# CaptainEven/DenseBox

Measured on AMD Instinct MI355X. Metric: training patches/sec (240x240), higher is better.
Workload: dtype f16; 1 GPU; full training step (fwd + fused dense loss w/ hard-negative mining + bwd + grad all-reduce + SGD) of DenseBoxLMLOC on 240x240 patches; net=DenseBoxLMLOC, batch_per_gpu=64, global_batch=64, patch=240x240, parallelism=dp1, half_neg=11, grad_finite=True

## Files before the change

densebox_amd/_lib.py:

```python
import ctypes as C
import os

_HERE = os.path.dirname(os.path.abspath(__file__))
LIB_PATH = os.environ.get('DBX_LIB') or os.path.join(_HERE, 'csrc', 'libdensebox_hip.so')

F16, BF16, F32 = 0, 1, 2
DTYPE_ID = {'f16': F16, 'bf16': BF16, 'f32': F32}
ESIZE = {F16: 2, BF16: 2, F32: 4}

EPI_BIAS, EPI_RELU, EPI_GATE, EPI_DROPMASK, EPI_ACCUM, EPI_F32_NCHW, EPI_DROPHASH = 1, 2, 4, 8, 16, 32, 64
CONV_WFRAG = 128
K_IGEMM, K_DMA, K_BAND, K_C64, K_C8, K_WS, K_P8 = 1, 2, 3, 4, 5, 6, 7


class View(C.Structure):
    _fields_ = [('ptr', C.c_void_p), ('n', C.c_int32), ('h', C.c_int32), ('w', C.c_int32),
                ('pad', C.c_int32), ('ld', C.c_int32), ('c_off', C.c_int32), ('c', C.c_int32)]


class ConvDesc(C.Structure):
    _fields_ = [('dtype', C.c_int32), ('kh', C.c_int32), ('kw', C.c_int32), ('cpad', C.c_int32),
                ('cin_pad', C.c_int32), ('cout_pad', C.c_int32), ('epilogue', C.c_int32), ('drop_seed', C.c_uint32)]


# ... 88 lines not shown
    'dbx_dp_destroy': (C.c_int, [_VP]),
    'dbx_conv_dgrad_wgrad1_scratch_bytes': (_I64, []),
    'dbx_conv_dgrad_wgrad1_fusable': (C.c_int, [_PC, _PV, _PV, _PV]),
    'dbx_conv_dgrad_wgrad1': (C.c_int, [_PC, _PV, _VP, _PV, _PV, _I32, _VP, _VP, _VP, _I32, _VP]),
    'dbx_conv_pool_fusable': (C.c_int, [_PC, _PV, _PV]),
    'dbx_conv_forward_pool': (C.c_int, [_PC, _PV, _VP, _VP, _PV, _PV, _I32, _VP]),
    'dbx_conv_forward_pool_idx': (C.c_int, [_PC, _PV, _VP, _VP, _PV, _PV, _I32, _VP, _VP]),
    'dbx_pack_weight': (C.c_int, [_I32, _I32, _VP, _I32, _I32, _I32, _I32, _VP, _I32, _I32, _I32, _I32, _VP]),
    'dbx_fold_heads': (C.c_int, [_VP, _VP, _VP, _VP, _I32, _VP, _VP, _VP]),
    'dbx_fold_refine': (C.c_int, [_VP, _VP, _VP, _VP, _VP, _VP, _I32, _I32, _VP, _VP, _VP, _VP]),
    'dbx_refine_eval': (C.c_int, [_VP, _VP, _I32, _I32, _I32, _VP, _VP, _VP, _VP]),
    'dbx_refine_backward_scratch_bytes': (C.c_int64, [_I32, _I32, _I32]),
    'dbx_refine_backward': (C.c_int, [_VP, _VP, _VP, _I32, _I32, _I32, _VP, _VP, _VP, _VP, _VP, _VP, _I32, _VP, _VP, _VP, _VP, _VP, _VP, _VP, _VP, _VP, _VP, _VP, _VP, _VP, _VP]),
    'dbx_upsample_bilinear_nchw_f32': (C.c_int, [_VP, _I32, _I32, _I32, _VP, _I32, _I32, _VP]),
    'dbx_pack_multi': (C.c_int, [_I32, _VP, _I32, _I64, _VP]),
    'dbx_sgd_pack_step': (C.c_int, [_I32, _VP, _I32, _I64, _VP, _F, _F, _F, _I32, _VP]),
    'dbx_head2_dgrad': (C.c_int, [_I32, _PV, C.POINTER(C.c_void_p), C.POINTER(C.c_int32), _I32, _PV, _VP, _I32, _I32, C.c_uint32, _VP]),
    'dbx_head2_wgrad_scratch_bytes': (_I64, [_I32, _I32]),
    'dbx_head2_wgrad': (C.c_int, [_I32, _PV, _PV, C.POINTER(C.c_int32), _I32, C.POINTER(C.c_void_p), C.POINTER(C.c_void_p), _VP, _VP]),
    'dbx_head2_backward': (C.c_int, [_I32, _PV, _PV, C.POINTER(C.c_void_p), C.POINTER(C.c_int32), _I32, _PV, _VP, _I32, _I32, C.c_uint32,
                                     C.POINTER(C.c_void_p), C.POINTER(C.c_void_p), _VP, _VP]),
    'dbx_head2_backward_up': (C.c_int, [_I32, _PV, _PV, C.POINTER(C.c_void_p), C.POINTER(C.c_int32), _I32, _PV, _VP, _I32, _I32, C.c_uint32,
                                        C.POINTER(C.c_void_p), C.POINTER(C.c_void_p), _VP, _PV, _VP]),
    'dbx_perspective_matrix': (C.c_int, [_VP, _VP, _VP]),
    'dbx_warp_perspective_u8': (C.c_int, [_VP, _I32, _I32, _I32, _VP, _VP, _I32, _I32, _VP]),
    'dbx_warp_batch_workspace_bytes': (_I64, [_I32]),
    'dbx_warp_perspective_batch_u8': (C.c_int, [C.POINTER(WarpJob), _I32, _I32, _VP, _VP, _VP]),
    'dbx_plate_crops_batch': (C.c_int, [_VP, _I32, _I32, _VP, _I64, _I64, _VP, _I32, _I32, _I32, _VP, _VP, _VP, _VP]),
    'dbx_match_gt_batch': (C.c_int, [_VP, _I32, _I64, _VP, _VP, _I32, _I32, _VP, _I32, _VP, _VP, _I32, _D, _VP, _VP, _VP, _VP, _VP, _VP]),
    'dbx_eval_append': (C.c_int, [_VP, _I32, _I64, _VP, _VP, _I32, _I32, _VP, _VP, _VP, _VP, _I64, _VP, _VP]),
    'dbx_track_update_batch': (C.c_int, [_VP, _I32, _I64, _VP, _VP, _I32, _I32, _VP, _VP, _I32, _I32, _I32, _D, _I32, _D, _D, _D, _VP, _VP, _VP,
                                         _VP, _VP, _VP]),
    'dbx_track_append': (C.c_int, [_VP, _VP, _I32, _I32, _I32, _VP, _I64, _VP, _VP]),
    'dbx_crop_sharpness': (C.c_int, [_VP, _I64, _I32, _I32, _I32, _VP, _VP]),
    'dbx_track_gallery_update': (C.c_int, [_VP, _VP, _VP, _VP, _VP, _VP, _VP, _VP, _VP, _VP, _VP, _VP, _VP, _I32, _I32, _I32, _I32, _I32, _I32,
                                           _I32, _I32, _I64, _I32, _D, _I32, _VP]),
    'dbx_draw_overlay_batch': (C.c_int, [_VP, _I32, _I32, _I32, _I32, _VP, _I32, _I64, _VP, _VP, _I32, _VP, _VP, _VP, _I32, _I32,
                                         C.POINTER(OverlayStyle), _VP]),
    'dbx_overlay_font': (C.c_int, [_VP]),
    'dbx_overlay_label': (C.c_int, [_D, _I32, C.c_char_p, _I32]),
    'dbx_resize_batch_workspace_bytes': (_I64, [_I32]),
    'dbx_resize_cubic_batch_u8': (C.c_int, [C.POINTER(ResizeJob), _I32, _I32, _VP, _VP, _VP]),
    'dbx_conv_wgrad_scratch_bytes': (_I64, [_I32, _PV, _PV, _I32, _I32]),
    'dbx_conv_wgrad': (C.c_int, [_I32, _PV, _PV, _I32, _I32, _I32, _I32, _I32, _VP, _VP, _VP, _I32, _VP]),
    'dbx_conv_wgrad_slice': (C.c_int, [_I32, _PV, _PV, _I32, _I32, _I32, _I32, _I32, _VP, _I32, _I32, _VP, _VP, _I32, _VP]),
    'dbx_conv_wgrad_pool_dz_ok': (C.c_int, [_I32, _PV, _PV, _I32, _I32]),
# ... 91 lines not shown
```

densebox_amd/csrc/aux_ops.hip:

```cpp
#include "common.hpp"
#include <mutex>

static thread_local char g_err[512] = "";
void dbx_set_error(const char* fmt, ...) {
    va_list ap;
    va_start(ap, fmt);
    vsnprintf(g_err, sizeof(g_err), fmt, ap);
    va_end(ap);
}
extern "C" const char* dbx_last_error(void) { return g_err; }
extern "C" int dbx_version(void) { return DBX_ABI_VERSION; }
extern "C" int dbx_device_arch(int device) {
    hipDeviceProp_t p;
    if (hipGetDeviceProperties(&p, device) != hipSuccess) { dbx_set_error("hipGetDeviceProperties failed"); return DBX_ERR_HIP; }
    int arch = 0;
    const char* s = p.gcnArchName;
    if (s[0] == 'g' && s[1] == 'f' && s[2] == 'x') arch = (int)strtol(s + 3, nullptr, 16) == 0x950 ? 950 : (int)strtol(s + 3, nullptr, 10);
    return arch;
}

template <typename T> struct Vec { static constexpr int N = 16 / sizeof(T); };

template <typename T> __device__ __forceinline__ void load_vec(const T* p, float (&v)[16 / sizeof(T)]) {
    const u32x4 raw = *(const u32x4*)p;
// ... 1036 lines not shown
extern "C" int dbx_head2_backward(int32_t dtype, const dbx_view* d_out, const dbx_view* hid, const float* const* w2, const int32_t* k,
                                  int32_t nh, const dbx_view* d_hid, const uint8_t* dropmask, int32_t dropmask_ld, int32_t use_hash,
                                  uint32_t drop_seed, float* const* dw, float* const* db, void* scratch, void* stream) {
    if (!d_out || !hid || !w2 || !k || !d_hid || !dw || !scratch) { dbx_set_error("head2_backward: null argument"); return DBX_ERR_ARG; }
    DBX_DISPATCH_DTYPE(dtype, head2_wgrad_t, d_out, hid, k, nh, dw, db, scratch, (hipStream_t)stream, w2, d_hid, dropmask, dropmask_ld,
                       use_hash, (unsigned)drop_seed);
}

#ifndef H2U_D
#define H2U_D 2
#endif
#ifndef H2U_NB
#define H2U_NB 4
#endif
#ifndef H2U_WGS
#define H2U_WGS 512
#endif
struct H2UHalf { int px_lo, px_n, own_lo, own_hi, ix_lo, ix_n; };
struct H2UPlan { int halves; H2UHalf h[2]; };
template <typename T, int KJ>
__global__ __launch_bounds__(256, 2) void head2_backward_up_kernel(FrameGeo dout, FrameGeo hid, FrameGeo dhid, FrameGeo dg, int hd0, int nhl, int slot,
                                                                   Head2Args ha, float* __restrict__ partial, float* __restrict__ bpartial,
                                                                   const unsigned char* __restrict__ mask, int mask_ld, int use_hash,
                                                                   unsigned drop_seed, float sy, float sx, H2UPlan plan, int nostore) {
    constexpr int V = 8, CS = 64, LPP = CS / V, D = H2U_D, PW = 32, NB = H2U_NB, NT = 6;
    static_assert(sizeof(T) == 2, "16-bit element types");
    __shared__ int s_x0[64], s_lo[32], s_hi[32];
    __shared__ float s_l0[64], s_l1[64];
    extern __shared__ __attribute__((aligned(16))) char h2u_smem[];
    float* const s_v = (float*)h2u_smem;
    const int nsl = nhl * (512 / CS), H = hid.h, W = hid.w;
    int b = blockIdx.x;
    const int sl = b % nsl; b /= nsl;
    const int half = b % plan.halves, grp = b / plan.halves, G = gridDim.x / (nsl * plan.halves);
    const H2UHalf hf = half ? plan.h[1] : plan.h[0];
    const int hd = hd0 + sl / (512 / CS), cbase = (sl % (512 / CS)) * CS;
    const int pl = threadIdx.x / LPP, ch = threadIdx.x % LPP, c0 = cbase + ch * V;
    const int px = hf.px_lo + pl;
    const bool active = pl < hf.px_n, owner = active && px >= hf.own_lo && px < hf.own_hi;
    if (threadIdx.x < W) {
        int x0, x1; float lx0, lx1;
        bilin_coef((int)threadIdx.x, sx, dg.w, x0, x1, lx0, lx1);
        s_x0[threadIdx.x] = x0; s_l0[threadIdx.x] = x1 == x0 ? lx0 + lx1 : lx0; s_l1[threadIdx.x] = x1 == x0 ? 0.f : lx1;
    }
    __syncthreads();
    if (threadIdx.x < hf.ix_n) {
        const int ix = hf.ix_lo + threadIdx.x;
// ... 206 lines not shown
            for (int j = 0; j < 8; ++j) red[4 * 8 * CS + wv * 8 + j] = j < KJ ? bs[j < KJ ? j : 0] : 0.f;
        }
    }
    __syncthreads();
    {
        const size_t blk = (size_t)grp * plan.halves + half;
        const int c = threadIdx.x % CS;
#pragma unroll
        for (int jj = 0; jj < 2; ++jj) {
            const int j = threadIdx.x / CS + 4 * jj;
            float o = 0.f;
#pragma unroll
            for (int q = 0; q < 4; ++q) o += red[(q * 8 + j) * CS + c];
            partial[(blk * nhl * 8 + (hd - hd0) * 8 + j) * 512 + cbase + c] = o;
        }
        if (cbase == 0 && threadIdx.x < 8) {
            float bsum = 0.f;
#pragma unroll
            for (int q = 0; q < 4; ++q) bsum += red[4 * 8 * CS + q * 8 + threadIdx.x];
            bpartial[blk * 32 + (hd - hd0) * 8 + threadIdx.x] = bsum;
        }
    }
}
static bool h2u_plan(int W, int ws, float sx, H2UPlan& p) {
    if (W > 64 || ws > 32 || W < 1 || ws < 1) return false;
    int x0[64];
    for (int ox = 0; ox < W; ++ox) { int v = (int)(sx * (float)ox); x0[ox] = v > ws - 1 ? ws - 1 : v; }
    if (W <= 32 && ws <= 16) { p.halves = 1; p.h[0] = p.h[1] = H2UHalf{0, W, 0, W, 0, ws}; return true; }
    const int S = ws / 2;
    if (S < 1 || S > 16 || ws - S > 16) return false;
    int hiL = -1, loR = W;
    for (int ox = 0; ox < W; ++ox) { if (x0[ox] <= S - 1) hiL = ox; if (x0[ox] >= S - 1 && ox < loR) loR = ox; }
    if (hiL + 1 > 32 || W - loR > 32 || loR > hiL + 1) return false;
    const int P = (loR + hiL + 1) / 2;
    p.halves = 2;
    p.h[0] = H2UHalf{0, hiL + 1, 0, P, 0, S};
    p.h[1] = H2UHalf{loR, W - loR, P, W, S, ws - S};
    return true;
}
template <typename T>
static int head2_backward_up_t(const dbx_view* dout, const dbx_view* hid, const float* const* w2, const int32_t* k, int nh, const dbx_view* dhid,
                               const uint8_t* mask, int mask_ld, int use_hash, unsigned drop_seed, float* const* dw, float* const* db,
                               void* scratch, const dbx_view* dg, hipStream_t s) {
    VIEW_VEC_CHECK(T, dg, "head2_backward_up d_g44");
    DBX_REQUIRE(dg->n == hid->n && dg->c == hid->c, "head2_backward_up: d_g44 has the hidden map's batch and channels");
    const float sy = ac_scale(dg->h, hid->h), sx = ac_scale(dg->w, hid->w);
    H2UPlan plan;
    bool fused = sizeof(T) == 2 && sy > 0.f && sy < 1.f && sx > 0.45f && sx < 1.f && hid->c % 64 == 0 && hid->h >= 2 && h2u_plan(hid->w, dg->w, sx, plan);
    if (const char* e = getenv("DBX_HEAD2_UP")) fused = fused && atoi(e) != 0;
    const bool nostore = dhid->ptr == nullptr;
    DBX_REQUIRE(!nostore || (fused && !mask), "head2_backward_up without d_hid: needs the one-pass kernel (dbx_head2_backward_up_fused) and hash / no dropout");
    if (!fused) {
        const int rc = head2_wgrad_t<T>(dout, hid, k, nh, dw, db, scratch, s, w2, dhid, mask, mask_ld, use_hash, drop_seed);
        return rc != DBX_OK ? rc : upsample_bwd_t<T>(dhid, dg, nullptr, s);
    }
    if constexpr (sizeof(T) == 2) {
        VIEW_VEC_CHECK(T, hid, "head2_backward_up hid");
        if (!nostore) VIEW_VEC_CHECK(T, dhid, "head2_backward_up d_hid");
        DBX_REQUIRE(nh >= 1 && nh <= 4 && hid->c == 512 * nh && dout->c % nh == 0 && dout->c / nh >= 8, "head2_backward_up: nh in 1..4, hid of 512*nh channels, d_out of nh slots >= 8 channels");
        DBX_REQUIRE(dout->n == hid->n && dout->h == hid->h && dout->w == hid->w && dhid->n == hid->n && dhid->h == hid->h && dhid->w == hid->w && dhid->c == hid->c,
                    "head2_backward_up: shape mismatch");
        DBX_REQUIRE(((size_t)dout->ptr % 16) == 0 && (dout->ld * sizeof(T)) % 16 == 0 && (dout->c_off * sizeof(T)) % 16 == 0 &&
                        ((dout->c / nh) * sizeof(T)) % 16 == 0, "head2_backward_up: d_out alignment");
        Head2Out o;
        Head2Args ha;
        ha.nh = nh; ha.slot = dout->c / nh;
        for (int i = 0; i < 4; ++i) {
            o.dw[i] = i < nh ? dw[i] : nullptr; o.db[i] = (i < nh && db) ? db[i] : nullptr; o.k[i] = i < nh ? k[i] : 0;
            ha.w2[i] = i < nh ? w2[i] : nullptr; ha.k[i] = i < nh ? k[i] : 0;
            if (i < nh) DBX_REQUIRE(k[i] >= 1 && k[i] <= 8 && dw[i] && w2[i] && ((size_t)w2[i] % 16) == 0, "head2_backward_up: k in 1..8, 16-byte aligned weights");
        }
        constexpr size_t smem = (size_t)2 * H2U_NB * 32 * 64 * 4;
        static_assert(smem >= (4 * 8 * 64 + 32) * 4 && 2 * smem + 4096 <= 160 * 1024, "LDS budget of two workgroups per CU");
        static DbxDevOnce attr_once; int attr_dev = 0;
        if (attr_once.pending(&attr_dev)) {
            DBX_HIP(hipFuncSetAttribute((const void*)head2_backward_up_kernel<T, 1>, hipFuncAttributeMaxDynamicSharedMemorySize, (int)smem));
            DBX_HIP(hipFuncSetAttribute((const void*)head2_backward_up_kernel<T, 2>, hipFuncAttributeMaxDynamicSharedMemorySize, (int)smem));
            DBX_HIP(hipFuncSetAttribute((const void*)head2_backward_up_kernel<T, 4>, hipFuncAttributeMaxDynamicSharedMemorySize, (int)smem));
            DBX_HIP(hipFuncSetAttribute((const void*)head2_backward_up_kernel<T, 8>, hipFuncAttributeMaxDynamicSharedMemorySize, (int)smem));
            attr_once.mark(attr_dev);
        }
        static int split = -1;
        if (split < 0) { const char* e = getenv("DBX_HEAD2_UP_SPLIT"); split = e ? atoi(e) : 1; }
        auto kup = [&](int kk) { return !split ? 8 : kk <= 1 ? 1 : kk <= 2 ? 2 : kk <= 4 ? 4 : 8; };
        float* const pbase = (float*)scratch;
        long long pused = 0;
        int blocks_max = 0;
        for (int h0 = 0; h0 < nh;) {
            int h1 = h0 + 1;
            while (h1 < nh && kup(k[h1]) == kup(k[h0])) ++h1;
            const int nhl = h1 - h0, nsl = nhl * 8, kj = kup(k[h0]);
            int groups = H2U_WGS / (nsl * plan.halves);
            groups = groups < 1 ? 1 : groups > hid->n ? hid->n : groups;
            const int blocks = groups * plan.halves;
            float* partial = pbase + pused;
            float* bpartial = partial + (size_t)blocks * nhl * 8 * 512;
            for (int i = h0; i < h1; ++i) { o.poff[i] = pused; o.boff[i] = pused + (long long)blocks * nhl * 8 * 512; o.nblk[i] = blocks; o.nhl[i] = nhl; o.hl[i] = i - h0; }
            pused += (long long)blocks * (nhl * 8 * 512 + 32);
            blocks_max = blocks > blocks_max ? blocks : blocks_max;
#define H2U_LAUNCH(KJ)                                                                                                              \
            hipLaunchKernelGGL((head2_backward_up_kernel<T, KJ>), dim3(blocks * nsl), dim3(256), smem, s, make_geo<T>(dout), make_geo<T>(hid),    \
                               make_geo<T>(nostore ? hid : dhid), make_geo<T>(dg), h0, nhl, dout->c / nh, ha, partial, bpartial, mask, mask_ld,    \
                               use_hash, drop_seed, sy, sx, plan, nostore ? 1 : 0)
            if (kj == 1) H2U_LAUNCH(1); else if (kj == 2) H2U_LAUNCH(2); else if (kj == 4) H2U_LAUNCH(4); else H2U_LAUNCH(8);
#undef H2U_LAUNCH
            DBX_LAUNCH_CHECK();
            h0 = h1;
        }
        for (int i = nh; i < 4; ++i) { o.poff[i] = 0; o.boff[i] = 0; o.nblk[i] = 0; o.nhl[i] = 1; o.hl[i] = 0; }
        float* partial = pbase; float* bpartial = pbase;
        const int blocks = blocks_max;
        const int total = nh * 8 * 512 + nh * 8;
        hipLaunchKernelGGL(head2_wgrad_reduce_kernel, dim3((total + 63) / 64), dim3(1024), 0, s, partial, bpartial, blocks, nh, o);
        DBX_LAUNCH_CHECK();
    }
    return DBX_OK;
}
template <typename T> static int head2_up_fused_t(const dbx_view* hid, const dbx_view* dg) {
    const float sy = ac_scale(dg->h, hid->h), sx = ac_scale(dg->w, hid->w);
    H2UPlan plan;
    bool fused = sizeof(T) == 2 && sy > 0.f && sy < 1.f && sx > 0.45f && sx < 1.f && hid->c % 64 == 0 && hid->h >= 2 && h2u_plan(hid->w, dg->w, sx, plan);
    if (const char* e = getenv("DBX_HEAD2_UP")) fused = fused && atoi(e) != 0;
    return fused ? 1 : 0;
}
extern "C" int dbx_head2_backward_up_fused(int32_t dtype, const dbx_view* hid, const dbx_view* d_g44) {
    if (!hid || !d_g44) return 0;
    switch (dtype) { case DBX_F16: return head2_up_fused_t<_Float16>(hid, d_g44); case DBX_BF16: return head2_up_fused_t<__bf16>(hid, d_g44); default: return 0; }
}
extern "C" int dbx_head2_backward_up(int32_t dtype, const dbx_view* d_out, const dbx_view* hid, const float* const* w2, const int32_t* k,
                                     int32_t nh, const dbx_view* d_hid, const uint8_t* dropmask, int32_t dropmask_ld, int32_t use_hash,
                                     uint32_t drop_seed, float* const* dw, float* const* db, void* scratch, const dbx_view* d_g44, void* stream) {
    if (!d_out || !hid || !w2 || !k || !d_hid || !dw || !scratch || !d_g44) { dbx_set_error("head2_backward_up: null argument"); return DBX_ERR_ARG; }
    DBX_DISPATCH_DTYPE(dtype, head2_backward_up_t, d_out, hid, w2, k, nh, d_hid, dropmask, dropmask_ld, use_hash, (unsigned)drop_seed, dw, db,
                       scratch, d_g44, (hipStream_t)stream);
}

struct PackJob { const float* src; void* dst; int co, ci, taps, mode; long long ktot; int cin_pad, row_off, k_off, rows_lim; };
template <typename T>
__global__ void pack_multi_kernel(const PackJob* __restrict__ jobs) {
    const PackJob j = jobs[blockIdx.y];
    const int total = j.co * j.ci * j.taps, taps = j.taps, ci = j.ci;
    T* wp = (T*)j.dst;
    const bool fwd = j.mode == 0 || j.mode == 4;
    const int rl = j.mode >= 4 ? (int)j.ktot : j.rows_lim;
    if (sizeof(T) == 2 && j.mode != 2 && (fwd ? ci : j.co) % 8 == 0 && (j.k_off & 7) == 0 && (j.cin_pad & 7) == 0 && taps <= 25) {
        __shared__ float tile[8][32 * 25];
        const int ot = (j.co + 7) / 8, ctn = (ci + 31) / 32, ntiles = ot * ctn, row_f = 32 * taps;
        for (int tl = blockIdx.x; tl < ntiles; tl += gridDim.x) {
            const int o0 = (tl / ctn) * 8, c0 = (tl % ctn) * 32;
            const int cw = min(32, ci - c0), ow = min(8, j.co - o0);
            __syncthreads();
            for (int e = threadIdx.x; e < 8 * row_f; e += blockDim.x) {
                const int r = e / row_f, f = e - r * row_f;
                tile[r][f] = (r < ow && f < cw * taps) ? j.src[((o0 + r) * ci + c0) * taps + f] : 0.f;
            }
            __syncthreads();
            const int nch = fwd ? 8 * taps * 4 : 32 * taps;
// ... 370 lines not shown
```

densebox_amd/engine.py:

```python
import ctypes as C
import os
import weakref

import torch

from . import _lib
from ._lib import View, ConvDesc, check, ptr, stream_ptr

_BACKBONE = [('conv1_1_1', 3, 64), ('conv1_2_1', 64, 64), ('conv2_1_1', 64, 128), ('conv2_2_1', 128, 128),
             ('conv3_1_1', 128, 256), ('conv3_2_1', 256, 256), ('conv3_4_1', 256, 256),
             ('conv4_1_1', 256, 512), ('conv4_2_1', 512, 512), ('conv4_3_1', 512, 512), ('conv4_4_1', 512, 512)]

_HEADS = {
    'DenseBox': [('det', 1), ('loc', 4)],
    'DenseBoxLM': [('det', 1), ('loc', 4), ('landmark', 4)],
    'DenseBoxLMLOC': [('det', 1), ('loc', 4), ('landmark', 4), ('lmloc', 8)],
}


_FWD_IO = {'conv1_1_1': ('x0', 'a11'), 'conv1_2_1': ('a11', 'a12'), 'conv2_1_1': ('p1', 'a21'), 'conv2_2_1': ('a21', 'a22'),
           'conv3_1_1': ('p2', 'a31'), 'conv3_2_1': ('a31', 'a32'), 'conv3_4_1': ('a32', 'c34'), 'conv4_1_1': ('p3', 'a41'),
           'conv4_2_1': ('a41', 'a42'), 'conv4_3_1': ('a42', 'a43'), 'conv4_4_1': ('a43', 'a44')}
_BWD_IO = {'conv4_4_1': ('d_a44', 'd_a43'), 'conv4_3_1': ('d_a43', 'd_a42'), 'conv4_2_1': ('d_a42', 'd_a41'),
           'conv4_1_1': ('d_a41', 'd_p3'), 'conv3_4_1': ('d_c34', 'd_a32'), 'conv3_2_1': ('d_a32', 'd_a31'),
# ... 1004 lines not shown
            dgrad('conv6_2_det', B['d_rf_2'].view(), B['d_rf_1'].view(), 5, 5, 4, 64, 64)
            conv_bwd('conv6_1_det', B['d_rf_1'].view(), B['rf_p'].view(), 3, 3, 0, 64, 5)
            dgrad('conv6_1_det', B['d_rf_1'].view(), B['d_rf_p'].view(), 3, 3, 2, 64, 64)
            check(L.dbx_maxpool2x2_bwd(dt, C.byref(B['rf_in'].view()), C.byref(B['d_rf_p'].view()),
                                       C.byref(B['d_rf_in'].view()), 0, 0, s))

        slot = {}
        srcs = []
        for i, (stem, k) in enumerate(heads):
            slot[stem] = B['d_out'].view(P.crf * i, P.crf)
            src = override.get(stem)
            srcs.append(src if src is not None else gout(stem, k))
        if override or kind == 'DenseBox':
            check(L.dbx_nchw_to_framed_slots(dt, (C.c_void_p * nh)(*[t.data_ptr() for t in srcs]), (C.c_int32 * nh)(*[k for _, k in heads]), nh, P.crf,
                                             C.byref(B['d_out'].view()), s))
        else:
            for (stem, k), t in zip(heads, srcs):
                check(L.dbx_nchw_to_framed(dt, ptr(t), k, C.byref(slot[stem]), s))
        if kind != 'DenseBox' and not override:
            check(L.dbx_framed_add_ch(dt, C.byref(B['d_rf_in'].view()), 0, 4, C.byref(slot['landmark']), 0, s))
            check(L.dbx_framed_add_ch(dt, C.byref(B['d_rf_in'].view()), 4, 1, C.byref(slot['det']), 0, s))

        hv = B['hid'].view()
        need = L.dbx_head2_wgrad_scratch_bytes(nh, hv.n * hv.h)
        if getattr(self, '_h2_scratch', None) is None or self._h2_scratch.numel() < need:
            self._h2_scratch = torch.empty(int(need), dtype=torch.uint8, device=dev)
        dw2 = [new_grad('conv5_2_%s.weight' % st) for st, _ in heads]
        db2 = [new_grad('conv5_2_%s.bias' % st) for st, _ in heads]
        prof = self.profile
        if prof is not None:
            ev0, ev1 = torch.cuda.Event(enable_timing=True), torch.cuda.Event(enable_timing=True)
            ev0.record()
        w2s = [self._param('conv5_2_%s.weight' % st).detach() for st, _ in heads]
        ks = (C.c_int32 * nh)(*[k for _, k in heads])
        h2_names = ['conv5_2_%s.weight' % st for st, _ in heads] + ['conv5_2_%s.bias' % st for st, _ in heads]
        mask_p = C.c_void_p(P.mask_buf.data_ptr()) if (P.drop_active and not P.drop_hash) else None
        hash_on, hash_seed = (1 if P.drop_hash else 0), (P.drop_seed if P.drop_hash else 0)
        lin = self._lin_bwd(dt)
        up_done = False
        gen = bool(getattr(P, 'heads_gen', False) and lin and side is None and mask_p is None)
        if gen and dt != _lib.F32:
            dhid_v = View(None, hv.n, hv.h, hv.w, 1, 512 * nh, 0, 512 * nh)
        else:
            dhid_v = self._d_hid(P).view()
        w2p = (C.c_void_p * nh)(*[w.data_ptr() for w in w2s])
        if side is not None:
            def run_h2():
                check(L.dbx_head2_wgrad(dt, C.byref(B['d_out'].view()), C.byref(hv), ks, nh,
                                        (C.c_void_p * nh)(*[t.data_ptr() for t in dw2]), (C.c_void_p * nh)(*[t.data_ptr() for t in db2]),
                                        ptr(self._h2_scratch), stream_ptr()))
                if sink is not None:
                    sink.ready(h2_names)
            on_side(run_h2)
            check(L.dbx_head2_dgrad(dt, C.byref(B['d_out'].view()), (C.c_void_p * nh)(*[w.data_ptr() for w in w2s]), ks, nh,
                                    C.byref(dhid_v), mask_p, 512 * nh, hash_on, hash_seed, s))
        elif lin:
            check(L.dbx_head2_backward_up(dt, C.byref(B['d_out'].view()), C.byref(hv), (C.c_void_p * nh)(*[w.data_ptr() for w in w2s]), ks, nh,
                                          C.byref(dhid_v), mask_p, 512 * nh, hash_on, hash_seed,
                                          (C.c_void_p * nh)(*[t.data_ptr() for t in dw2]), (C.c_void_p * nh)(*[t.data_ptr() for t in db2]),
                                          ptr(self._h2_scratch), C.byref(B['d_g44'].view()), s))
            up_done = True
            if gen and dt == _lib.F32:
                bh = P.B['d_hid']
                P.ws[bh.off:bh.off + bh.bytes].view(torch.float32).fill_(float('nan'))
        else:
            check(L.dbx_head2_backward(dt, C.byref(B['d_out'].view()), C.byref(hv), (C.c_void_p * nh)(*[w.data_ptr() for w in w2s]), ks, nh,
                                       C.byref(dhid_v), mask_p, 512 * nh, hash_on, hash_seed,
                                       (C.c_void_p * nh)(*[t.data_ptr() for t in dw2]), (C.c_void_p * nh)(*[t.data_ptr() for t in db2]),
                                       ptr(self._h2_scratch), s))
            if sink is not None:
                sink.ready(h2_names)
        if prof is not None:
            ev1.record()
            prof.append({'kernel': ('head2_backward_up_kernel<%s>' if up_done else 'head2_wgrad_kernel<%s>') % ('f16', 'bf16', 'f32')[dt],
                         'flops': 2.0 * hv.n * hv.h * hv.w * 512 * sum(k for _, k in heads) * (1 if side is not None else 2), 'start': ev0, 'end': ev1})
        w1n = ['conv5_1_%s.weight' % st for st, _ in heads]
        b1n = ['conv5_1_%s.bias' % st for st, _ in heads]
        if sink is not None:
            dw1, db1 = sink.region(w1n).view(512 * nh, 768, 1, 1), sink.region(b1n)
        else:
            dw1 = torch.empty((512 * nh, 768, 1, 1), dtype=torch.float32, device=dev)
            db1 = torch.empty((512 * nh,), dtype=torch.float32, device=dev)
        c34 = B['fusion'].view(512, 256)
# ... 134 lines not shown
```

include/densebox_hip.h:

```cpp
#ifndef DENSEBOX_HIP_H
#define DENSEBOX_HIP_H

#include <stdint.h>

#ifdef __cplusplus
extern "C" {
#endif

enum dbx_status {
    DBX_OK = 0,
    DBX_ERR_ARG = -1,
    DBX_ERR_HIP = -2,
    DBX_ERR_DTYPE = -3
};

enum dbx_dtype { DBX_F16 = 0, DBX_BF16 = 1, DBX_F32 = 2 };

const char* dbx_last_error(void);
#define DBX_ABI_VERSION 13
int dbx_version(void);
int dbx_device_arch(int device);

typedef struct dbx_view {
    void*   ptr;
// ... 57 lines not shown
int dbx_conv_forward_pool_idx(const dbx_conv_desc* d, const dbx_view* x, const void* w_packed, const float* bias,
                              const dbx_view* y, const dbx_view* ypool, int32_t write_full, void* idx, void* stream);

int dbx_pack_weight(int32_t dtype, int32_t mode, const float* w_oihw, int32_t co, int32_t ci, int32_t kh, int32_t kw,
                    void* w_packed, int32_t rows_pad, int32_t cin_pad, int32_t row_off, int32_t k_off, void* stream);

int dbx_pack_multi(int32_t dtype, const void* jobs, int32_t count, int64_t max_elems, void* stream);

int dbx_sgd_pack_step(int32_t dtype, const void* jobs, int32_t count, int64_t max_elems, float* const* ptrs, float lr, float momentum,
                      float weight_decay, int32_t first_step, void* stream);

int dbx_head2_dgrad(int32_t dtype, const dbx_view* d_out, const float* const* w2, const int32_t* k, int32_t nh,
                    const dbx_view* d_hid, const uint8_t* dropmask, int32_t dropmask_ld, int32_t use_hash, uint32_t drop_seed,
                    void* stream);
int64_t dbx_head2_wgrad_scratch_bytes(int32_t nh, int32_t rows);
int dbx_head2_wgrad(int32_t dtype, const dbx_view* d_out, const dbx_view* hid, const int32_t* k, int32_t nh,
                    float* const* dw, float* const* db, void* scratch, void* stream);
int dbx_head2_backward(int32_t dtype, const dbx_view* d_out, const dbx_view* hid, const float* const* w2, const int32_t* k,
                       int32_t nh, const dbx_view* d_hid, const uint8_t* dropmask, int32_t dropmask_ld, int32_t use_hash,
                       uint32_t drop_seed, float* const* dw, float* const* db, void* scratch, void* stream);
int dbx_head2_backward_up(int32_t dtype, const dbx_view* d_out, const dbx_view* hid, const float* const* w2, const int32_t* k,
                          int32_t nh, const dbx_view* d_hid, const uint8_t* dropmask, int32_t dropmask_ld, int32_t use_hash,
                          uint32_t drop_seed, float* const* dw, float* const* db, void* scratch, const dbx_view* d_g44, void* stream);
int dbx_conv_wgrad_pool_dz_ok(int32_t dtype, const dbx_view* dz, const dbx_view* x, int32_t kh, int32_t kw);
int dbx_conv_wgrad_pool_dz(int32_t dtype, const dbx_view* dy, const void* idx, int32_t idx_channels, const dbx_view* dz, const dbx_view* x,
                           int32_t kh, int32_t kw, int32_t cpad, int32_t co, int32_t ci, float* dw_oihw, float* db, void* scratch,
                           int32_t accumulate, int32_t write_dz, void* stream);
int dbx_head2_backward_up_fused(int32_t dtype, const dbx_view* hid, const dbx_view* d_g44);
int dbx_heads1_wgrad_gen_ok(int32_t dtype, const dbx_view* x, int32_t nh);
int dbx_heads1_wgrad_gen(int32_t dtype, const dbx_view* d_out, const dbx_view* x, const float* const* w2, const int32_t* k, int32_t nh,
                         int32_t use_hash, uint32_t drop_seed, int32_t ci, float* dw_oihw, int32_t dw_ci_total, int32_t dw_ci_off,
                         float* db, void* scratch, void* stream);
int dbx_heads1_dgrad_gen(int32_t dtype, const dbx_view* d_out, const float* const* w2, const int32_t* k, int32_t nh, int32_t use_hash,
                         uint32_t drop_seed, const void* w1t_frag, const dbx_view* y, const dbx_view* gate, void* stream);

int dbx_fold_heads(const float* w2, const float* b2, const float* w1, const float* b1, int32_t k, float* w_out,
                   float* b_out, void* stream);
int dbx_fold_refine(const float* w1, const float* b1, const float* w2, const float* b2, const float* w3, const float* b3,
                    int32_t ci, int32_t cm, float* w_out, float* b_out, float* v_out, void* stream);
int dbx_refine_eval(const float* landmark_nchw, const float* score_nchw, int32_t n, int32_t h, int32_t w, const float* w_fold,
                    const float* b_fold, float* out_small, void* stream);
int dbx_upsample_bilinear_nchw_f32(const float* x, int32_t planes, int32_t hi, int32_t wi, float* y, int32_t ho, int32_t wo,
                                   void* stream);
int64_t dbx_refine_backward_scratch_bytes(int32_t n, int32_t h, int32_t w);
int dbx_refine_backward(const float* d_refine, const float* landmark, const float* score, int32_t n, int32_t h, int32_t w,
                        const float* w1, const float* b1, const float* w2, const float* b2, const float* w3, const float* b3,
// ... 235 lines not shown
```

Measured before the change: 7528 patches/s.

## Add sparse row-gated head2 backward for loc heads with nonzero gradient pixels

Adds a flag pass that marks pixels where the loc/lmloc head output gradients are nonzero, then (when the nonzero fraction is small) skips the dense fused head2 backward blocks for those heads and runs sparse kernels. These accumulate wgrad only over flagged pixels and compute the upsampled input gradient only where flagged outputs contribute. It targets wasted dense work, since hard-negative-mined loc losses leave most gradient pixels zero. It adds extra launches, a flags buffer and a runtime fallback decision, plus a slow per-pixel serial consume loop in the sparse wgrad.

```diff
diff --git a/densebox_amd/_lib.py b/densebox_amd/_lib.py
--- a/densebox_amd/_lib.py
+++ b/densebox_amd/_lib.py
@@ -134,6 +134,9 @@
                                      C.POINTER(C.c_void_p), C.POINTER(C.c_void_p), _VP, _VP]),
     'dbx_head2_backward_up': (C.c_int, [_I32, _PV, _PV, C.POINTER(C.c_void_p), C.POINTER(C.c_int32), _I32, _PV, _VP, _I32, _I32, C.c_uint32,
                                         C.POINTER(C.c_void_p), C.POINTER(C.c_void_p), _VP, _PV, _VP]),
+    'dbx_head2_backward_up_rows_scratch_bytes': (_I64, [_I32, _I32, _I32, _I32]),
+    'dbx_head2_backward_up_rows': (C.c_int, [_I32, _PV, _PV, C.POINTER(C.c_void_p), C.POINTER(C.c_int32), _I32, _PV, _VP, _I32, _I32, C.c_uint32,
+                                             C.POINTER(C.c_void_p), C.POINTER(C.c_void_p), _VP, _PV, C.c_uint32, _VP]),
     'dbx_perspective_matrix': (C.c_int, [_VP, _VP, _VP]),
     'dbx_warp_perspective_u8': (C.c_int, [_VP, _I32, _I32, _I32, _VP, _VP, _I32, _I32, _VP]),
     'dbx_warp_batch_workspace_bytes': (_I64, [_I32]),
diff --git a/densebox_amd/csrc/aux_ops.hip b/densebox_amd/csrc/aux_ops.hip
--- a/densebox_amd/csrc/aux_ops.hip
+++ b/densebox_amd/csrc/aux_ops.hip
@@ -1082,7 +1082,9 @@
 __global__ __launch_bounds__(256, 2) void head2_backward_up_kernel(FrameGeo dout, FrameGeo hid, FrameGeo dhid, FrameGeo dg, int hd0, int nhl, int slot,
                                                                    Head2Args ha, float* __restrict__ partial, float* __restrict__ bpartial,
                                                                    const unsigned char* __restrict__ mask, int mask_ld, int use_hash,
-                                                                   unsigned drop_seed, float sy, float sx, H2UPlan plan, int nostore) {
+                                                                   unsigned drop_seed, float sy, float sx, H2UPlan plan, int nostore,
+                                                                   const int* __restrict__ gate, int gcand) {
+    if (gate && (gcand >> (hd0 + (int)(blockIdx.x % (unsigned)(nhl * 8)) / 8) & 1) && gate[1] == 0) return;
     constexpr int V = 8, CS = 64, LPP = CS / V, D = H2U_D, PW = 32, NB = H2U_NB, NT = 6;
     static_assert(sizeof(T) == 2, "16-bit element types");
     __shared__ int s_x0[64], s_lo[32], s_hi[32];
@@ -1335,6 +1337,296 @@
         }
     }
 }
+struct Head2Cand { int hd[4]; int n; };
+template <typename T>
+__global__ __launch_bounds__(256) void head2_rows_flag_kernel(FrameGeo dout, int slot, Head2Cand cd, unsigned char* __restrict__ flags,
+                                                              int* __restrict__ status, int npix) {
+    static_assert(sizeof(T) == 2, "16-bit element types");
+    const int m = blockIdx.x * 256 + threadIdx.x;
+    bool f = false;
+    if (m < npix) {
+        const int x = m % dout.w, r = m / dout.w, y = r % dout.h, n = r / dout.h;
+        const T* g = (const T*)dout.base + geo_pix(dout, n, y, x);
+        for (int q = 0; q < cd.n; ++q)
+            for (int c = 0; c < slot; c += 8) {
+                const u32x4 v = *(const u32x4*)(g + cd.hd[q] * slot + c);
+                f = f || (((v.x | v.y | v.z | v.w) & 0x7FFF7FFFu) != 0u);
+            }
+        flags[m] = f ? 1 : 0;
+    }
+    const unsigned long long b = __ballot(f);
+    if ((threadIdx.x & 63) == 0 && b) atomicAdd(&status[0], __popcll(b));
+}
+__global__ void head2_rows_status_kernel(int* __restrict__ status, int npix) { status[1] = status[0] > npix / 8 ? 1 : 0; }
+struct Head2RowsPlan { int hd[4], G[4], nhl[4], hl[4], wg0[5]; long long poff[4], boff[4]; int n; };
+template <typename T>
+__global__ __launch_bounds__(256) void head2_rows_wgrad_kernel(FrameGeo dout, FrameGeo hid, int slot, Head2RowsPlan rp, H2UPlan plan,
+                                                               const unsigned char* __restrict__ flags, const int* __restrict__ status,
+                                                               float* __restrict__ pbase) {
+    if (status[1]) return;
+    static_assert(sizeof(T) == 2, "16-bit element types");
+    constexpr int V = 8, CS = 64, LPP = CS / V, CH = 128;
+    __shared__ unsigned short s_mask[256];
+    __shared__ unsigned long long s_nz[4];
+    __shared__ int s_list[CH];
+    __shared__ u32x4 s_g[CH], s_h[CH][LPP];
+    __shared__ float s_red[4 * 8 * CS + 32];
+    int ci = 0;
+#pragma unroll
+    for (int q = 1; q < 4; ++q) if (q < rp.n && (int)blockIdx.x >= rp.wg0[q]) ci = q;
+    int hd = rp.hd[0], G = rp.G[0], nhl = rp.nhl[0], hl = rp.hl[0], wg0 = rp.wg0[0];
+    long long poff = rp.poff[0], boff = rp.boff[0];
+#pragma unroll
+    for (int q = 1; q < 4; ++q)
+        if (ci == q) { hd = rp.hd[q]; G = rp.G[q]; nhl = rp.nhl[q]; hl = rp.hl[q]; wg0 = rp.wg0[q]; poff = rp.poff[q]; boff = rp.boff[q]; }
+    const int wl = (int)blockIdx.x - wg0, sl = wl % 8, blk = wl / 8, half = blk % plan.halves, grp = blk / plan.halves;
+    const H2UHalf hf = half ? plan.h[1] : plan.h[0];
+    const int cbase = sl * CS, pl = threadIdx.x / LPP, ch = threadIdx.x % LPP, px = hf.px_lo + pl;
+    const bool owner = pl < hf.px_n && px >= hf.own_lo && px < hf.own_hi;
+    const int lane = threadIdx.x & 63, wv = threadIdx.x >> 6;
+    const int HW = hid.h * hid.w;
+    typedef float f32x2 __attribute__((ext_vector_type(2)));
+    f32x2 acc[8][V / 2];
+    float bs[8];
+#pragma unroll
+    for (int j = 0; j < 8; ++j) {
+        bs[j] = 0.f;
+#pragma unroll
+        for (int i = 0; i < V / 2; ++i) acc[j][i] = (f32x2){0.f, 0.f};
+    }
+    for (int img = grp; img < hid.n; img += G) {
+        const unsigned char* fl = flags + (size_t)img * HW;
+        for (int base = 0; base < HW; base += 4096) {
+            unsigned mk = 0;
+#pragma unroll
+            for (int i = 0; i < 16; ++i) {
+                const int p = base + threadIdx.x * 16 + i;
+                if (p < HW && fl[p]) mk |= 1u << i;
+            }
+            __syncthreads();
+            s_mask[threadIdx.x] = (unsigned short)mk;
+            const unsigned long long nzb = __ballot(mk != 0);
+            if (lane == 0) s_nz[wv] = nzb;
+            __syncthreads();
+            int cnt = 0;
+            auto consume = [&]() {
+                __syncthreads();
+#pragma unroll
+                for (int it = 0; it < (CH * (LPP + 1) + 255) / 256; ++it) {
+                    const int e = it * 256 + (int)threadIdx.x, q = e / (LPP + 1), part = e % (LPP + 1);
+                    if (q < cnt) {
+                        const int p = s_list[q], y = p / hid.w, x = p - y * hid.w;
+                        if (part < LPP) s_h[q][part] = *(const u32x4*)((const T*)hid.base + geo_pix(hid, img, y, x) + hd * 512 + cbase + part * V);
+                        else s_g[q] = *(const u32x4*)((const T*)dout.base + geo_pix(dout, img, y, x) + hd * slot);
+                    }
+                }
+                __syncthreads();
+                for (int q = 0; q < cnt; ++q) {
+                    const int p = s_list[q], x = p % hid.w;
+                    if (owner && x == px) {
+                        const u32x4 graw = s_g[q], hraw = s_h[q][ch];
+                        const T* ge = (const T*)&graw;
+                        const T* he = (const T*)&hraw;
+                        float h[V];
+#pragma unroll
+                        for (int i = 0; i < V; ++i) h[i] = to_f32(he[i]);
+#pragma unroll
+                        for (int j = 0; j < 8; ++j) {
+                            const float gj = to_f32(ge[j]);
+                            bs[j] += gj;
+                            const f32x2 g2 = {gj, gj};
+#pragma unroll
+                            for (int i = 0; i < V / 2; ++i) acc[j][i] = g2 * (f32x2){h[2 * i], h[2 * i + 1]} + acc[j][i];
+                        }
+                    }
+                }
+                __syncthreads();
+                cnt = 0;
+            };
+            for (int q4 = 0; q4 < 4; ++q4) {
+                unsigned long long nz = s_nz[q4];
+                while (nz) {
+                    const int t = q4 * 64 + __ffsll((long long)nz) - 1;
+                    nz &= nz - 1;
+                    unsigned m16 = s_mask[t];
+                    while (m16) {
+                        const int p = base + t * 16 + __ffs((int)m16) - 1;
+                        m16 &= m16 - 1;
+                        if (threadIdx.x == 0) s_list[cnt] = p;
+                        if (++cnt == CH) consume();
+                    }
+                }
+            }
+            if (cnt) consume();
+        }
+    }
+#pragma unroll
+    for (int j = 0; j < 8; ++j) {
+#pragma unroll
+        for (int i = 0; i < V; ++i) {
+            float a = acc[j][i >> 1][i & 1];
+            a += __shfl_xor(a, 8); a += __shfl_xor(a, 16); a += __shfl_xor(a, 32);
+            acc[j][i >> 1][i & 1] = a;
+        }
+        float bsum = bs[j];
+        bsum += __shfl_xor(bsum, 8); bsum += __shfl_xor(bsum, 16); bsum += __shfl_xor(bsum, 32);
+        bs[j] = bsum;
+    }
+    __syncthreads();
+    if (lane < LPP) {
+#pragma unroll
+        for (int j = 0; j < 8; ++j) {
+            *(f32x4*)&s_red[(wv * 8 + j) * CS + lane * V] = (f32x4){acc[j][0][0], acc[j][0][1], acc[j][1][0], acc[j][1][1]};
+            *(f32x4*)&s_red[(wv * 8 + j) * CS + lane * V + 4] = (f32x4){acc[j][2][0], acc[j][2][1], acc[j][3][0], acc[j][3][1]};
+        }
+        if (lane == 0) {
+#pragma unroll
+            for (int j = 0; j < 8; ++j) s_red[4 * 8 * CS + wv * 8 + j] = bs[j];
+        }
+    }
+    __syncthreads();
+    {
+        float* const partial = pbase + poff;
+        float* const bpartial = pbase + boff;
+        const int c = threadIdx.x % CS;
+#pragma unroll
+        for (int jj = 0; jj < 2; ++jj) {
+            const int j = threadIdx.x / CS + 4 * jj;
+            float o = 0.f;
+#pragma unroll
+            for (int q = 0; q < 4; ++q) o += s_red[(q * 8 + j) * CS + c];
+            partial[((size_t)blk * nhl * 8 + hl * 8 + j) * 512 + cbase + c] = o;
+        }
+        if (cbase == 0 && threadIdx.x < 8) {
+            float bsum = 0.f;
+#pragma unroll
+            for (int q = 0; q < 4; ++q) bsum += s_red[4 * 8 * CS + q * 8 + threadIdx.x];
+            bpartial[(size_t)blk * 32 + hl * 8 + threadIdx.x] = bsum;
+        }
+    }
+}
+template <typename T>
+__global__ __launch_bounds__(256) void head2_rows_dg_kernel(FrameGeo dout, FrameGeo dg, int H, int W, Head2Args ha, Head2Cand cd,
+                                                            const unsigned char* __restrict__ flags, const int* __restrict__ status,
+                                                            int use_hash, unsigned drop_seed, float sy, float sx) {
+    if (status[1]) return;
+    static_assert(sizeof(T) == 2, "16-bit element types");
+    constexpr int V = 8;
+    const int lane = threadIdx.x & 63;
+    const long long total = (long long)dg.n * dg.h * dg.w;
+    long long sp = (long long)blockIdx.x * 4 + (threadIdx.x >> 6);
+    if (sp >= total) return;
+    const int ix = (int)(sp % dg.w); sp /= dg.w;
+    const int iy = (int)(sp % dg.h), img = (int)(sp / dg.h);
+    int oy_lo = H, oy_hi = -1, ox_lo = W, ox_hi = -1;
+    for (int base = 0; base < H; base += 64) {
+        const int oy = base + lane;
+        int y0, y1; float l0, l1;
+        bilin_coef(oy < H ? oy : H - 1, sy, dg.h, y0, y1, l0, l1);
+        const unsigned long long hit = __ballot(oy < H && (y0 == iy || y1 == iy));
+        if (hit) { if (oy_hi < 0) oy_lo = base + __ffsll((long long)hit) - 1; oy_hi = base + 63 - __clzll((long long)hit); }
+    }
+    for (int base = 0; base < W; base += 64) {
+        const int ox = base + lane;
+        int x0, x1; float l0, l1;
+        bilin_coef(ox < W ? ox : W - 1, sx, dg.w, x0, x1, l0, l1);
+        const unsigned long long hit = __ballot(ox < W && (x0 == ix || x1 == ix));
+        if (hit) { if (ox_hi < 0) ox_lo = base + __ffsll((long long)hit) - 1; ox_hi = base + 63 - __clzll((long long)hit); }
+    }
+    const int ny = oy_hi - oy_lo + 1, nx = ox_hi - ox_lo + 1;
+    const unsigned char* fl = flags + (size_t)img * H * W;
+    bool any = false;
+    if (ny <= 8 && nx <= 8) {
+        const int r = lane >> 3, q = lane & 7;
+        const bool in = r < ny && q < nx;
+        const unsigned char f = fl[in ? (oy_lo + r) * W + ox_lo + q : 0];
+        any = __ballot(in && f) != 0ull;
+    } else {
+        for (int oy = oy_lo; oy <= oy_hi; ++oy)
+            for (int base = ox_lo; base <= ox_hi; base += 64) {
+                const int ox = base + lane;
+                const unsigned char f = fl[ox <= ox_hi ? oy * W + ox : oy * W + ox_hi];
+                const unsigned long long hit = __ballot(ox <= ox_hi && f);
+                any = any || hit != 0ull;
+            }
+    }
+    const int c0 = lane * V;
+    T* const pix = (T*)dg.base + geo_pix(dg, img, iy, ix) + c0;
+    if (!any) {
+#pragma unroll
+        for (int ci = 0; ci < 4; ++ci)
+            if (ci < cd.n) *(u32x4*)(pix + cd.hd[ci] * 512) = (u32x4){0u, 0u, 0u, 0u};
+        return;
+    }
+    for (int ci = 0; ci < cd.n; ++ci) {
+        int hd = cd.hd[0];
+#pragma unroll
+        for (int q = 1; q < 4; ++q) if (ci == q) hd = cd.hd[q];
+        T* const out = pix + hd * 512;
+        const float* wp = ha.w2[0];
+        int k = ha.k[0];
+#pragma unroll
+        for (int hh = 1; hh < 4; ++hh)
+            if (hd == hh && ha.w2[hh]) { wp = ha.w2[hh]; k = ha.k[hh]; }
+        const float dscale = use_hash ? 2.f : 1.f;
+        float acc[V];
+#pragma unroll
+        for (int i = 0; i < V; ++i) acc[i] = 0.f;
+        for (int ox = ox_lo; ox <= ox_hi; ++ox) {
+            int x0, x1; float lx0, lx1;
+            bilin_coef(ox, sx, dg.w, x0, x1, lx0, lx1);
+            const float cx = x0 == ix ? (x1 == x0 ? lx0 + lx1 : lx0) : lx1;
+            float v[V];
+#pragma unroll
+            for (int i = 0; i < V; ++i) v[i] = 0.f;
+            bool col = false;
+            for (int oy = oy_lo; oy <= oy_hi; ++oy) {
+                if (!fl[oy * W + ox]) continue;
+                col = true;
+                int y0, y1; float ly0, ly1;
+                bilin_coef(oy, sy, dg.h, y0, y1, ly0, ly1);
+                const float cy = (y0 == iy ? ly0 : 0.f) + (y1 == iy ? ly1 : 0.f);
+                const u32x4 graw = *(const u32x4*)((const T*)dout.base + geo_pix(dout, img, oy, ox) + hd * ha.slot);
+                const T* ge = (const T*)&graw;
+                float o[V];
+#pragma unroll
+                for (int i = 0; i < V; ++i) o[i] = 0.f;
+#pragma unroll
+                for (int j = 0; j < 8; ++j) {
+                    if (j >= k) break;
+                    const float gj = to_f32(ge[j]);
+                    const f32x4 wa = *(const f32x4*)(wp + (size_t)j * 512 + c0), wb = *(const f32x4*)(wp + (size_t)j * 512 + c0 + 4);
+                    const float wj[V] = {wa.x, wa.y, wa.z, wa.w, wb.x, wb.y, wb.z, wb.w};
+#pragma unroll
+                    for (int i = 0; i < V; ++i) o[i] = fmaf(gj, to_f32(from_f32<T>(wj[i])) * dscale, o[i]);
+                }
+                if (use_hash) {
+                    const unsigned m = (unsigned)(((long long)img * H + oy) * W + ox);
+                    const unsigned kb8 = dbx_drop_hash32(drop_seed, m, (unsigned)(hd * 512 + c0) >> 5) >> ((unsigned)c0 & 31u);
+#pragma unroll
+                    for (int i = 0; i < V; ++i) o[i] = (kb8 >> i & 1u) ? o[i] : 0.f;
+                }
+#pragma unroll
+                for (int i = 0; i < V; ++i) v[i] = fmaf(cy, to_f32(from_f32<T>(o[i])), v[i]);
+            }
+            if (col) {
+#pragma unroll
+                for (int i = 0; i < V; ++i) acc[i] = fmaf(cx, v[i], acc[i]);
+            }
+        }
+        u32x4 raw;
+        T* oe = (T*)&raw;
+#pragma unroll
+        for (int i = 0; i < V; ++i) oe[i] = from_f32<T>(acc[i]);
+        *(u32x4*)out = raw;
+    }
+}
+static int64_t head2_rows_dense_bytes(int nh, int n, int h) { return (dbx_head2_wgrad_scratch_bytes(nh, n * h) + 255) / 256 * 256; }
+extern "C" int64_t dbx_head2_backward_up_rows_scratch_bytes(int32_t nh, int32_t n, int32_t h, int32_t w) {
+    if (nh < 1 || nh > 4 || n < 1 || h < 1 || w < 1) return 0;
+    const int64_t npix = (int64_t)n * h * w;
+    return head2_rows_dense_bytes(nh, n, h) + (npix + 255) / 256 * 256 + 256;
+}
 static bool h2u_plan(int W, int ws, float sx, H2UPlan& p) {
     if (W > 64 || ws > 32 || W < 1 || ws < 1) return false;
     int x0[64];
@@ -1354,7 +1646,7 @@
 template <typename T>
 static int head2_backward_up_t(const dbx_view* dout, const dbx_view* hid, const float* const* w2, const int32_t* k, int nh, const dbx_view* dhid,
                                const uint8_t* mask, int mask_ld, int use_hash, unsigned drop_seed, float* const* dw, float* const* db,
-                               void* scratch, const dbx_view* dg, hipStream_t s) {
+                               void* scratch, const dbx_view* dg, hipStream_t s, bool rows = false, unsigned cand = 0) {
     VIEW_VEC_CHECK(T, dg, "head2_backward_up d_g44");
     DBX_REQUIRE(dg->n == hid->n && dg->c == hid->c, "head2_backward_up: d_g44 has the hidden map's batch and channels");
     const float sy = ac_scale(dg->h, hid->h), sx = ac_scale(dg->w, hid->w);
@@ -1363,6 +1655,7 @@
     if (const char* e = getenv("DBX_HEAD2_UP")) fused = fused && atoi(e) != 0;
     const bool nostore = dhid->ptr == nullptr;
     DBX_REQUIRE(!nostore || (fused && !mask), "head2_backward_up without d_hid: needs the one-pass kernel (dbx_head2_backward_up_fused) and hash / no dropout");
+    DBX_REQUIRE(!rows || (nostore && cand < (1u << nh)), "head2_backward_up_rows: needs the one-pass form without a stored d_hid (d_hid->ptr == NULL) and candidates among the nh heads");
     if (!fused) {
         const int rc = head2_wgrad_t<T>(dout, hid, k, nh, dw, db, scratch, s, w2, dhid, mask, mask_ld, use_hash, drop_seed);
         return rc != DBX_OK ? rc : upsample_bwd_t<T>(dhid, dg, nullptr, s);
@@ -1399,6 +1692,25 @@
         float* const pbase = (float*)scratch;
         long long pused = 0;
         int blocks_max = 0;
+        const int* gate = nullptr;
+        const unsigned char* flags = nullptr;
+        Head2Cand cd{};
+        Head2RowsPlan rp{};
+        if (cand) {
+            const long long npix = (long long)hid->n * hid->h * hid->w;
+            DBX_REQUIRE(npix < (1ll << 31), "head2_backward_up_rows: more than 2^31 pixels");
+            unsigned char* const fl = (unsigned char*)scratch + head2_rows_dense_bytes(nh, hid->n, hid->h);
+            int* const status = (int*)(fl + (npix + 255) / 256 * 256);
+            for (int i = 0; i < nh; ++i)
+                if (cand >> i & 1) cd.hd[cd.n++] = i;
+            gate = status; flags = fl;
+            DBX_HIP(hipMemsetAsync(status, 0, 16, s));
+            hipLaunchKernelGGL(head2_rows_flag_kernel<T>, dim3((unsigned)((npix + 255) / 256)), dim3(256), 0, s, make_geo<T>(dout), dout->c / nh, cd,
+                               fl, status, (int)npix);
+            DBX_LAUNCH_CHECK();
+            hipLaunchKernelGGL(head2_rows_status_kernel, dim3(1), dim3(1), 0, s, status, (int)npix);
+            DBX_LAUNCH_CHECK();
+        }
         for (int h0 = 0; h0 < nh;) {
             int h1 = h0 + 1;
             while (h1 < nh && kup(k[h1]) == kup(k[h0])) ++h1;
@@ -1409,16 +1721,34 @@
             float* partial = pbase + pused;
             float* bpartial = partial + (size_t)blocks * nhl * 8 * 512;
             for (int i = h0; i < h1; ++i) { o.poff[i] = pused; o.boff[i] = pused + (long long)blocks * nhl * 8 * 512; o.nblk[i] = blocks; o.nhl[i] = nhl; o.hl[i] = i - h0; }
+            bool has_cand = false;
+            for (int i = h0; i < h1; ++i)
+                if (cand >> i & 1) {
+                    const int q = rp.n++;
+                    rp.hd[q] = i; rp.G[q] = groups; rp.nhl[q] = nhl; rp.hl[q] = i - h0; rp.poff[q] = o.poff[i]; rp.boff[q] = o.boff[i];
+                    rp.wg0[q + 1] = rp.wg0[q] + blocks * 8;
+                    has_cand = true;
+                }
             pused += (long long)blocks * (nhl * 8 * 512 + 32);
             blocks_max = blocks > blocks_max ? blocks : blocks_max;
 #define H2U_LAUNCH(KJ)                                                                                                              \
             hipLaunchKernelGGL((head2_backward_up_kernel<T, KJ>), dim3(blocks * nsl), dim3(256), smem, s, make_geo<T>(dout), make_geo<T>(hid),    \
                                make_geo<T>(nostore ? hid : dhid), make_geo<T>(dg), h0, nhl, dout->c / nh, ha, partial, bpartial, mask, mask_ld,    \
-                               use_hash, drop_seed, sy, sx, plan, nostore ? 1 : 0)
+                               use_hash, drop_seed, sy, sx, plan, nostore ? 1 : 0, has_cand ? gate : (const int*)nullptr, (int)cand)
             if (kj == 1) H2U_LAUNCH(1); else if (kj == 2) H2U_LAUNCH(2); else if (kj == 4) H2U_LAUNCH(4); else H2U_LAUNCH(8);
 #undef H2U_LAUNCH
             DBX_LAUNCH_CHECK();
             h0 = h1;
+        }
+        if (cand) {
+            hipLaunchKernelGGL(head2_rows_wgrad_kernel<T>, dim3((unsigned)rp.wg0[rp.n]), dim3(256), 0, s, make_geo<T>(dout), make_geo<T>(hid),
+                               dout->c / nh, rp, plan, flags, gate, pbase);
+            DBX_LAUNCH_CHECK();
+            const long long waves = (long long)dg->n * dg->h * dg->w;
+            DBX_REQUIRE((waves + 3) / 4 < (1ll << 31), "head2_backward_up_rows: d_g44 too large");
+            hipLaunchKernelGGL(head2_rows_dg_kernel<T>, dim3((unsigned)((waves + 3) / 4)), dim3(256), 0, s, make_geo<T>(dout), make_geo<T>(dg), hid->h,
+                               hid->w, ha, cd, flags, gate, use_hash, drop_seed, sy, sx);
+            DBX_LAUNCH_CHECK();
         }
         for (int i = nh; i < 4; ++i) { o.poff[i] = 0; o.boff[i] = 0; o.nblk[i] = 0; o.nhl[i] = 1; o.hl[i] = 0; }
         float* partial = pbase; float* bpartial = pbase;
@@ -1446,6 +1776,21 @@
     if (!d_out || !hid || !w2 || !k || !d_hid || !dw || !scratch || !d_g44) { dbx_set_error("head2_backward_up: null argument"); return DBX_ERR_ARG; }
     DBX_DISPATCH_DTYPE(dtype, head2_backward_up_t, d_out, hid, w2, k, nh, d_hid, dropmask, dropmask_ld, use_hash, (unsigned)drop_seed, dw, db,
                        scratch, d_g44, (hipStream_t)stream);
+}
+template <typename T>
+static int head2_backward_up_rows_t(const dbx_view* dout, const dbx_view* hid, const float* const* w2, const int32_t* k, int nh, const dbx_view* dhid,
+                                    const uint8_t* mask, int mask_ld, int use_hash, unsigned drop_seed, float* const* dw, float* const* db,
+                                    void* scratch, const dbx_view* dg, unsigned cand, hipStream_t s) {
+    if constexpr (sizeof(T) != 2) { dbx_set_error("head2_backward_up_rows: 16-bit types only"); return DBX_ERR_ARG; }
+    else return head2_backward_up_t<T>(dout, hid, w2, k, nh, dhid, mask, mask_ld, use_hash, drop_seed, dw, db, scratch, dg, s, true, cand);
+}
+extern "C" int dbx_head2_backward_up_rows(int32_t dtype, const dbx_view* d_out, const dbx_view* hid, const float* const* w2, const int32_t* k,
+                                          int32_t nh, const dbx_view* d_hid, const uint8_t* dropmask, int32_t dropmask_ld, int32_t use_hash,
+                                          uint32_t drop_seed, float* const* dw, float* const* db, void* scratch, const dbx_view* d_g44,
+                                          uint32_t cand_mask, void* stream) {
+    if (!d_out || !hid || !w2 || !k || !d_hid || !dw || !scratch || !d_g44) { dbx_set_error("head2_backward_up_rows: null argument"); return DBX_ERR_ARG; }
+    DBX_DISPATCH_DTYPE(dtype, head2_backward_up_rows_t, d_out, hid, w2, k, nh, d_hid, dropmask, dropmask_ld, use_hash, (unsigned)drop_seed, dw, db,
+                       scratch, d_g44, (unsigned)cand_mask, (hipStream_t)stream);
 }
 
 struct PackJob { const float* src; void* dst; int co, ci, taps, mode; long long ktot; int cin_pad, row_off, k_off, rows_lim; };
diff --git a/densebox_amd/engine.py b/densebox_amd/engine.py
--- a/densebox_amd/engine.py
+++ b/densebox_amd/engine.py
@@ -1050,7 +1050,7 @@
             check(L.dbx_framed_add_ch(dt, C.byref(B['d_rf_in'].view()), 4, 1, C.byref(slot['det']), 0, s))
 
         hv = B['hid'].view()
-        need = L.dbx_head2_wgrad_scratch_bytes(nh, hv.n * hv.h)
+        need = max(L.dbx_head2_wgrad_scratch_bytes(nh, hv.n * hv.h), L.dbx_head2_backward_up_rows_scratch_bytes(nh, hv.n, hv.h, hv.w))
         if getattr(self, '_h2_scratch', None) is None or self._h2_scratch.numel() < need:
             self._h2_scratch = torch.empty(int(need), dtype=torch.uint8, device=dev)
         dw2 = [new_grad('conv5_2_%s.weight' % st) for st, _ in heads]
@@ -1083,10 +1083,15 @@
             check(L.dbx_head2_dgrad(dt, C.byref(B['d_out'].view()), (C.c_void_p * nh)(*[w.data_ptr() for w in w2s]), ks, nh,
                                     C.byref(dhid_v), mask_p, 512 * nh, hash_on, hash_seed, s))
         elif lin:
-            check(L.dbx_head2_backward_up(dt, C.byref(B['d_out'].view()), C.byref(hv), (C.c_void_p * nh)(*[w.data_ptr() for w in w2s]), ks, nh,
-                                          C.byref(dhid_v), mask_p, 512 * nh, hash_on, hash_seed,
-                                          (C.c_void_p * nh)(*[t.data_ptr() for t in dw2]), (C.c_void_p * nh)(*[t.data_ptr() for t in db2]),
-                                          ptr(self._h2_scratch), C.byref(B['d_g44'].view()), s))
+            h2_args = (dt, C.byref(B['d_out'].view()), C.byref(hv), (C.c_void_p * nh)(*[w.data_ptr() for w in w2s]), ks, nh,
+                       C.byref(dhid_v), mask_p, 512 * nh, hash_on, hash_seed,
+                       (C.c_void_p * nh)(*[t.data_ptr() for t in dw2]), (C.c_void_p * nh)(*[t.data_ptr() for t in db2]),
+                       ptr(self._h2_scratch), C.byref(B['d_g44'].view()))
+            if gen and dt != _lib.F32 and os.environ.get('DBX_HEAD_ROWS', '1') != '0':
+                rows_mask = sum(1 << i for i, (st, _) in enumerate(heads) if st in ('loc', 'lmloc'))
+                check(L.dbx_head2_backward_up_rows(*h2_args, rows_mask, s))
+            else:
+                check(L.dbx_head2_backward_up(*h2_args, s))
             up_done = True
             if gen and dt == _lib.F32:
                 bh = P.B['d_hid']
diff --git a/include/densebox_hip.h b/include/densebox_hip.h
--- a/include/densebox_hip.h
+++ b/include/densebox_hip.h
@@ -103,6 +103,11 @@
 int dbx_head2_backward_up(int32_t dtype, const dbx_view* d_out, const dbx_view* hid, const float* const* w2, const int32_t* k,
                           int32_t nh, const dbx_view* d_hid, const uint8_t* dropmask, int32_t dropmask_ld, int32_t use_hash,
                           uint32_t drop_seed, float* const* dw, float* const* db, void* scratch, const dbx_view* d_g44, void* stream);
+int64_t dbx_head2_backward_up_rows_scratch_bytes(int32_t nh, int32_t n, int32_t h, int32_t w);
+int dbx_head2_backward_up_rows(int32_t dtype, const dbx_view* d_out, const dbx_view* hid, const float* const* w2, const int32_t* k,
+                               int32_t nh, const dbx_view* d_hid, const uint8_t* dropmask, int32_t dropmask_ld, int32_t use_hash,
+                               uint32_t drop_seed, float* const* dw, float* const* db, void* scratch, const dbx_view* d_g44,
+                               uint32_t cand_mask, void* stream);
 int dbx_conv_wgrad_pool_dz_ok(int32_t dtype, const dbx_view* dz, const dbx_view* x, int32_t kh, int32_t kw);
 int dbx_conv_wgrad_pool_dz(int32_t dtype, const dbx_view* dy, const void* idx, int32_t idx_channels, const dbx_view* dz, const dbx_view* x,
                            int32_t kh, int32_t kw, int32_t cpad, int32_t co, int32_t ci, float* dw_oihw, float* db, void* scratch,
```

Result: no change. 7498 patches/s (-0.4%).
